# fedelopez77/sympa

Measured on AMD Instinct MI355X. Metric: pairwise Siegel distances/sec (upper, riem, n=4), higher is better.
Workload: dtype f64; 1 GPU; upper-riem-n4-b65536; manifold=upper, dist_metric=riem, dims=4, nodes=5041, table=trained, pairs=sampled, launch=fused, api=Model.forward_batches(Model.prepare_batches(list of K batches)), streams=1, parallelism=pairs sharded rank::1, table replicated, no collective, steps_per_launch=32

## Files before the change

__graft_entry__.py:

```python
import os
import subprocess
import sys

ROOT = os.path.dirname(os.path.abspath(__file__))
CSRC = os.path.join(ROOT, "sympa_amd", "csrc")
HOSTSIM = os.path.join(ROOT, "tests", "hostsim")
if ROOT not in sys.path:
    sys.path.insert(0, ROOT)


def _stale(target, sources):
    if not os.path.exists(target):
        return True
    t = os.path.getmtime(target)
    return any(os.path.getmtime(s) > t for s in sources)


INSTANCE_LIST = "siegel_bwd_instances.hpp"
INSTANCE_FAMILIES = {
    "COOP": ("siegel_bwd_coop_instance.hip", "siegel_bwd_coop_{model}_{n}_{form}"),
    "HALF": ("siegel_bwd_half_instance.hip", "siegel_bwd_half_{model}_{n}_{form}"),
    "SPLIT_SPECTRAL": ("siegel_bwd_split_instance.hip", "siegel_bwd_split_spectral_{model}_{n}"),
    "SPLIT_GRADIENT": ("siegel_bwd_split_instance.hip", "siegel_bwd_split_gradient_{model}_{n}_{form}"),
    "ONE_LANE": ("siegel_bwd_one_lane_instance.hip", "siegel_bwd_n{n}_{model}_{form}"),
}


def bwd_instances():
    import re
    out = []
    for line in open(os.path.join(CSRC, INSTANCE_LIST)):
        if line.startswith("SYMPA_BWD_"):
            m = re.fullmatch(r"SYMPA_BWD_([A-Z_]+)\(([a-z]+), (\d+)(?:, ([a-z]+))?\)\n", line)
            if not m or m.group(1) not in INSTANCE_FAMILIES or \
                    (m.group(4) is None) != ("{form}" not in INSTANCE_FAMILIES[m.group(1)][1]):
                raise ValueError(f"{INSTANCE_LIST}: cannot read the line {line!r}")
            out.append((m.group(1), m.group(2), int(m.group(3)), m.group(4)))
    return out


def hip_units():
    sources = {src for src, _ in INSTANCE_FAMILIES.values()}
    units = [(f, f, []) for f in os.listdir(CSRC) if f.endswith(".hip") and f not in sources]
    for family, model, n, form in bwd_instances():
        src, name = INSTANCE_FAMILIES[family]
        defines = [f"-DSYMPA_INST_MODEL={model}", f"-DSYMPA_INST_N={n}"] + ([f"-DSYMPA_INST_FORM={form}"] if form else [])
        units.append((name.format(model=model, n=n, form=form), src, defines))
    return sorted(units)


def build_hip(force=False):
    import shutil
    import tempfile
    from concurrent.futures import ThreadPoolExecutor
    sys.path.insert(0, os.path.join(ROOT, "tools"))
    import asm_stats
    import check_dpp_hazards
    import dma_reload_check
    import json
    so = os.path.join(CSRC, "libsympa_hip.so")
    units = hip_units()

    def obj_name(u):
        return (u[:-4] if u.endswith(".hip") else u) + ".o"
    headers = [os.path.join(CSRC, f) for f in os.listdir(CSRC) if f.endswith(".hpp")]
    headers.append(os.path.join(ROOT, "include", "sympa_hip.h"))
    flags = ["--offload-arch=gfx950", "-O3", "-std=c++17", "-fPIC"]
    unit_flags = {"siegel_dist_big.hip": ["-mllvm", "-enable-misched=0"],
                  "siegel_dist_big_dual.hip": ["-mllvm", "-enable-misched=0"],
                  "siegel_packed.hip": ["-mllvm", "-enable-misched=0"]}
    stats_units = ("siegel_dist.hip", "siegel_dist_big.hip", "siegel_packed.hip", "spd.hip")
    stats_path = os.path.join(CSRC, "asm_stats.json")
    try:
        stats = json.load(open(stats_path))
    except (OSError, ValueError):
        stats = {}
    report_path = os.path.join(CSRC, "dpp_hazard_report.txt")
    report = {}
    if os.path.exists(report_path):
        for line in open(report_path):
            parts = line.split()
            if len(parts) >= 2 and not line.startswith("#"):
                report[parts[0]] = line.strip()

    dma = {}

    def dma_note(u):
        return f"; {dma[u][0]} LDS-DMA instructions, {dma[u][1]} behind a scratch reload" if u in dma else ""

    def compile_checked(u, src, extra):
        tmp = tempfile.mkdtemp(prefix="sympa_build_")
        try:
            obj = os.path.join(tmp, obj_name(u))
            subprocess.check_call(["hipcc"] + flags + unit_flags.get(u, []) + extra + ["-c", "--save-temps=obj", "-o", obj, src], cwd=CSRC,
                                  stderr=subprocess.DEVNULL)
            asm = [os.path.join(tmp, f) for f in os.listdir(tmp) if f.endswith("gfx950.s")]
            assert len(asm) == 1, f"{u}: expected one gfx950 assembly file, got {asm}"
            total, bad = check_dpp_hazards.check_file(asm[0])
            dma[u] = dma_reload_check.totals(asm[0])
            if u in stats_units:
                stats[u] = asm_stats.kernel_flop_mix(asm[0])
            shutil.move(obj, os.path.join(CSRC, obj_name(u)))
            return total, bad
        finally:
            shutil.rmtree(tmp, ignore_errors=True)

    retries = [(["-DSYMPA_COOP_NOP_IN_ASM"], "SYMPA_COOP_NOP_IN_ASM")]

    def compile_unit(unit):
        u, src, defines = unit
        src, obj = os.path.join(CSRC, src), os.path.join(CSRC, obj_name(u))
        if force or u not in report or "LDS-DMA" not in report[u] or (u in stats_units and u not in stats) or \
                _stale(obj, [src] + headers):
            total, bad = compile_checked(u, src, defines)
            if bad:
                first = bad[0]
                print(f"[build] {u}: DPP hazard in the generated code ({first[1]}  ->  {first[2]})", flush=True)
                for extra, label in retries:
                    total, bad2 = compile_checked(u, src, defines + extra)
                    if not bad2:
                        report[u] = f"{u} {total} DPP instructions, {len(bad)} hazards -> rebuilt with {label}, clean" + dma_note(u)
                        break
                else:
                    raise RuntimeError(f"{u}: DPP hazard even with SYMPA_COOP_NOP_IN_ASM: {bad2[0]}")
            else:
                report[u] = f"{u} {total} DPP instructions, clean" + dma_note(u)
        return obj

    with ThreadPoolExecutor(max_workers=min(8, len(units))) as ex:
        objs = list(ex.map(compile_unit, units))
    with open(report_path, "w") as f:
        f.write("# tools/check_dpp_hazards.py and tools/dma_reload_check.py over the gfx950 assembly of every translation unit "
                "(written by build())\n")
        for u, _, _ in units:
            f.write(report[u] + "\n")
    with open(stats_path, "w") as f:
        json.dump({u: stats[u] for u in stats_units if u in stats}, f, indent=1, sort_keys=True)
    if force or _stale(so, objs):
        subprocess.check_call(["hipcc"] + flags + ["-shared", "-o", so] + objs, cwd=CSRC)
    return so


def build_torch_binding(force=False):
    import sysconfig
    import torch
    from torch.utils import cpp_extension as ce
    src = os.path.join(CSRC, "torch_binding.cpp")
    out = os.path.join(ROOT, "sympa_amd", "_fast" + sysconfig.get_config_var("EXT_SUFFIX"))
    stamp = out + ".torch_version"
    built_for = open(stamp).read().strip() if os.path.exists(stamp) else ""
    want = f"{torch.__version__} cxx11abi={int(torch.compiled_with_cxx11_abi())}"
    if not (force or built_for != want or _stale(out, [src, os.path.join(ROOT, "include", "sympa_hip.h")])):
        return out
    tl = os.path.join(os.path.dirname(torch.__file__), "lib")
    cmd = ["g++", "-O2", "-std=c++17", "-fPIC", "-shared", "-D__HIP_PLATFORM_AMD__=1", "-DUSE_ROCM=1",
           "-DTORCH_EXTENSION_NAME=_fast", "-DTORCH_API_INCLUDE_EXTENSION_H",
           f"-D_GLIBCXX_USE_CXX11_ABI={int(torch.compiled_with_cxx11_abi())}",
           "-I" + sysconfig.get_paths()["include"], "-I/opt/rocm/include"] + ["-I" + p for p in ce.include_paths()] + \
          [src, "-o", out, "-L" + tl, "-lc10", "-lc10_hip", "-ltorch", "-ltorch_cpu", "-ltorch_hip", "-ltorch_python",
           "-Wl,-rpath," + tl]
    subprocess.check_call(cmd, cwd=ROOT)
    with open(stamp, "w") as f:
        f.write(want + "\n")
    return out


def build_hostsim(force=False):
    so = os.path.join(HOSTSIM, "libsympa_hostsim.so")
    srcs = [os.path.join(HOSTSIM, "hostsim.cpp"), os.path.join(CSRC, "siegel_math.hpp"),
            os.path.join(CSRC, "siegel_math_bwd.hpp"), os.path.join(CSRC, "siegel_math_bwd_split.hpp"),
            os.path.join(CSRC, "siegel_table_math.hpp"),
            os.path.join(CSRC, "siegel_math_generic.hpp"), os.path.join(CSRC, "spd_math.hpp"),
            os.path.join(CSRC, "spd_math_bwd.hpp"), os.path.join(CSRC, "tridiag_invit.hpp")]
    if force or _stale(so, srcs):
        subprocess.check_call(["g++", "-O2", "-std=c++17", "-shared", "-fPIC", "-o", so, srcs[0]], cwd=HOSTSIM)
    return so


def build() -> None:
    build_hip()
    try:
        build_torch_binding()
    except (subprocess.CalledProcessError, OSError, ImportError) as e:
        print(f"[build] thin torch binding NOT built ({e!r}); the ctypes binding serves Model.forward", flush=True)
    build_hostsim()
    import sympa_amd
    from sympa_amd import _lib
    lib = _lib.load()
    assert lib.sympa_max_dims() >= 8
    print("built:", lib.sympa_version().decode())


def smoke() -> None:
    import torch
    build_hip()
    from oracle import siegel_oracle as so
    from sympa_amd import ops
    from sympa_amd.model import Model

    assert torch.cuda.is_available(), "smoke() needs a GPU"
    dev = torch.device("cuda:0")
    g = torch.Generator().manual_seed(7)
    n, N, b = 4, 97, 500
    for model in ("upper", "bounded"):
        class A:
            manifold, metric, dims, num_points = model, "riem", n, N
            scale_coef, scale_init, train_scale = 1.0, 1.0, False
        m = Model(A)
        with torch.no_grad():
            x = 0.3 * torch.randn(N, n, n, generator=g); x = 0.5 * (x + x.transpose(-1, -2))
            a = 0.3 * torch.randn(N, n, n, generator=g); y = torch.matrix_exp(0.5 * (a + a.transpose(-1, -2)))
            pts = torch.stack((x, 0.5 * (y + y.transpose(-1, -2))), 1)
            if model == "bounded":
                pts = so.to_symmetric(so.cayley_transform(pts))
            m.embeddings.embeds.data = pts
        m = m.to(dev)
        trip = torch.stack((torch.randint(0, N, (b,), generator=g), torch.randint(0, N, (b,), generator=g),
                            torch.randint(1, 9, (b,), generator=g)), 1)
        with torch.no_grad():
            got = m(trip.to(dev)).cpu()
        ops.check_status(dev)
        want = so.model_forward(pts, trip, model, "riem")
        rel = (((got - want).abs() - 1e-12).clamp_min(0) / want.abs().clamp_min(1e-300)).max().item()
        raw_abs = (got - want).abs().max().item()
        nz = want.abs() > 1e-9
        raw_rel = ((got - want).abs()[nz] / want.abs()[nz]).max().item()
        assert rel < 1e-8, f"{model}: HIP vs oracle rel err {rel}"
        print(f"smoke {model}: b={b} n={n} HIP vs oracle: max abs err {raw_abs:.2e}, max rel err {raw_rel:.2e} "
              f"(over the {int(nz.sum())} pairs with d > 1e-9), {rel:.2e} after the 1e-12 absolute floor")
    n8, N8 = 8, 61

    class A8:
        manifold, metric, dims, num_points = "upper", "riem", n8, N8
        scale_coef, scale_init, train_scale = 1.0, 1.0, False
    m = Model(A8)
    with torch.no_grad():
        x = 0.3 * torch.randn(N8, n8, n8, generator=g); x = 0.5 * (x + x.transpose(-1, -2))
        a = 0.2 * torch.randn(N8, n8, n8, generator=g); y = torch.matrix_exp(0.5 * (a + a.transpose(-1, -2)))
        pts = torch.stack((x, 0.5 * (y + y.transpose(-1, -2))), 1)
        m.embeddings.embeds.data = pts
    m = m.to(dev)
    trips = [torch.stack((torch.randint(0, N8, (bb,), generator=g), torch.randint(0, N8, (bb,), generator=g)), 1) for bb in (4100, 130, 1)]
    with torch.no_grad():
        outs = [o.cpu() for o in m.forward_batches([t.to(dev) for t in trips])]
    ops.check_status(dev)
    assert m.packed_table() is not None and m.packed_table().repacks == 1, "the packed path did not run"
    rel = 0.0
    for t, o in zip(trips, outs):
        want = so.model_forward(pts, t, "upper", "riem")
        rel = max(rel, (((o - want).abs() - 1e-12).clamp_min(0) / want.abs().clamp_min(1e-300)).max().item())
    assert rel < 1e-8, f"packed n = 8: HIP vs oracle rel err {rel}"
    print(f"smoke upper n={n8} packed list form (3 batches, {sum(t.shape[0] for t in trips)} pairs): HIP vs oracle max rel err {rel:.2e}")


if __name__ == "__main__":
    build()
    if len(sys.argv) > 1 and sys.argv[1] == "smoke":
        smoke()
```

sympa_amd/csrc/siegel_math.hpp:

```cpp
#pragma once

#include <cmath>
#include <cstdint>

#if defined(__HIPCC__)
#define SYMPA_HD __host__ __device__ __forceinline__
#else
#define SYMPA_HD inline
#endif

#ifndef SYMPA_UNROLL
#define SYMPA_UNROLL _Pragma("unroll")
#endif

namespace sympa {

enum Model : int { MODEL_UPPER = 0, MODEL_BOUNDED = 1, MODEL_DUAL = 2 };
enum Metric : int { METRIC_RIEM = 0, METRIC_FONE = 1, METRIC_FINF = 2, METRIC_FMIN = 3, METRIC_WSUM = 4 };

enum StatusBit : int { ST_NOT_PD = 1, ST_NONFINITE = 2, ST_BAD_INDEX = 4, ST_NO_CONVERGENCE = 8 };

#if defined(__HIP_DEVICE_COMPILE__)
SYMPA_HD bool wave_all(bool p) { return __all(p ? 1 : 0) != 0; }
SYMPA_HD double seed_rsq(double x) { return __builtin_amdgcn_rsq(x); }
SYMPA_HD double seed_rcp(double x) { return __builtin_amdgcn_rcp(x); }
SYMPA_HD double d_frexp_mant(double x) { return __builtin_amdgcn_frexp_mant(x); }
SYMPA_HD int d_frexp_exp(double x) { return __builtin_amdgcn_frexp_exp(x); }
#else
SYMPA_HD bool wave_all(bool p) { return p; }
SYMPA_HD double seed_rsq(double x) { return (1.0 / std::sqrt(x)) * (1.0 + 4.0e-8); }
SYMPA_HD double seed_rcp(double x) { return (1.0 / x) * (1.0 - 4.0e-8); }
SYMPA_HD double d_frexp_mant(double x) { int e; return std::frexp(x, &e); }
SYMPA_HD int d_frexp_exp(double x) { int e; (void)std::frexp(x, &e); return e; }
#endif
SYMPA_HD double d_fma(double a, double b, double c) { return __builtin_fma(a, b, c); }
SYMPA_HD bool d_finite(double x) { return fabs(x) <= 1.79e308; }

SYMPA_HD double d_rsqrt(double x) {
    const double y = seed_rsq(x);
    const double e = d_fma(-(x * y), y, 1.0);
    return d_fma(y, e * d_fma(0.375, e, 0.5), y);
}
SYMPA_HD double d_rcp(double x) {
    const double y = seed_rcp(x);
    const double e = d_fma(-x, y, 1.0);
    return d_fma(y, d_fma(e, e, e), y);
}
constexpr double TINY = 1e-300;
SYMPA_HD double d_sqrt(double x) { return x * d_rsqrt(x + TINY); }

SYMPA_HD double d_log1p(double u) {
    const double x = 1.0 + u;
    double m = d_frexp_mant(x);
    int k = d_frexp_exp(x);
    const bool lowhalf = m < 0.70710678118654752440;
    m = lowhalf ? 2.0 * m : m;
    k = lowhalf ? k - 1 : k;
    const bool small = u < 0.4;
    const double f = small ? u : m - 1.0;
    const double kd = small ? 0.0 : (double)k;
    const double s = f * d_rcp(2.0 + f);
    const double z = s * s;
    double r = 1.479819860511658591e-01;
    r = d_fma(r, z, 1.531383769920937332e-01);
    r = d_fma(r, z, 1.818357216161805012e-01);
    r = d_fma(r, z, 2.222219843214978396e-01);
    r = d_fma(r, z, 2.857142874366239149e-01);
    r = d_fma(r, z, 3.999999999940941908e-01);
    r = d_fma(r, z, 6.666666666666735130e-01);
    r = r * z;
    const double l = d_fma(-s, f - r, f);
    return d_fma(kd, 6.93147180559945286227e-01, l);
}

SYMPA_HD double d_atan2_pos(double s, double c) {
    const bool swap = s > c;
    const double num = swap ? c : s;
    const double den = swap ? s : c;
    const bool big = num > 0.41421356237309503 * den;
    const double xn = big ? num - den : num;
    const double xd = big ? num + den : den;
    const double x = xn * d_rcp(xd);
    const double z = x * x;
    const double w = z * z;
    double s1 = 1.62858201153657823623e-02;
    s1 = d_fma(s1, w, 4.97687799461593236017e-02);
    s1 = d_fma(s1, w, 6.66107313738753120669e-02);
    s1 = d_fma(s1, w, 9.09088713343650656196e-02);
    s1 = d_fma(s1, w, 1.42857142725034663711e-01);
    s1 = d_fma(s1, w, 3.33333333333329318027e-01);
    s1 = s1 * z;
    double s2 = -3.65315727442169155270e-02;
    s2 = d_fma(s2, w, -5.83357013379057348645e-02);
    s2 = d_fma(s2, w, -7.69187620504482999495e-02);
    s2 = d_fma(s2, w, -1.11111104054623557880e-01);
    s2 = d_fma(s2, w, -1.99999999998764832476e-01);
    s2 = s2 * w;
    double a = d_fma(-x, s1 + s2, x);
    a = big ? 7.85398163397448278999e-01 + (a + 3.06161699786838301793e-17) : a;
    return swap ? 1.57079632679489655800e+00 + (6.12323399573676603587e-17 - a) : a;
}

template <int N>
struct CMat {
    double re[N][N];
    double im[N][N];
};

template <int N, bool COMPLEX>
struct Tri {
    double re[N][N];
    double im[N][N];
    double rdiag[N];
};

template <int N>
SYMPA_HD void load_point(const double* __restrict__ p, CMat<N>& z) {
SYMPA_UNROLL
    for (int i = 0; i < N; ++i) {
SYMPA_UNROLL
        for (int j = 0; j < N; ++j) {
            z.re[i][j] = p[(i <= j) ? i * N + j : j * N + i];
            z.im[i][j] = p[N * N + ((i <= j) ? i * N + j : j * N + i)];
        }
    }
}

template <int N>
SYMPA_HD bool chol_real(const double (&y)[N][N], Tri<N, false>& l) {
    bool ok = true;
SYMPA_UNROLL
    for (int j = 0; j < N; ++j) {
        double s = y[j][j];
SYMPA_UNROLL
        for (int k = 0; k < j; ++k) s = d_fma(-l.re[j][k], l.re[j][k], s);
        ok = ok && (s > 0.0);
        const double r = d_rsqrt(s);
        l.rdiag[j] = r;
SYMPA_UNROLL
        for (int i = j + 1; i < N; ++i) {
            double t = y[j][i];
SYMPA_UNROLL
            for (int k = 0; k < j; ++k) t = d_fma(-l.re[i][k], l.re[j][k], t);
            l.re[i][j] = t * r;
        }
    }
    return ok;
}

template <bool PLUS>
SYMPA_HD double wwh_sign(double x) {
    if constexpr (PLUS) return x;
    else return -x;
}
template <int N, bool PLUS>
SYMPA_HD bool chol_id_pm_wwh(const CMat<N>& w, Tri<N, true>& c) {
    bool ok = true;
SYMPA_UNROLL
    for (int j = 0; j < N; ++j) {
        double s = 1.0;
SYMPA_UNROLL
        for (int l = 0; l < N; ++l) {
            s = d_fma(wwh_sign<PLUS>(w.re[j][l]), w.re[j][l], s);
            s = d_fma(wwh_sign<PLUS>(w.im[j][l]), w.im[j][l], s);
        }
SYMPA_UNROLL
        for (int k = 0; k < j; ++k) {
            s = d_fma(-c.re[j][k], c.re[j][k], s);
            s = d_fma(-c.im[j][k], c.im[j][k], s);
        }
        ok = ok && (s > 0.0);
        const double r = d_rsqrt(s);
        c.rdiag[j] = r;
SYMPA_UNROLL
        for (int i = j + 1; i < N; ++i) {
            double tr = 0.0, ti = 0.0;
SYMPA_UNROLL
            for (int l = 0; l < N; ++l) {
                tr = d_fma(wwh_sign<PLUS>(w.re[i][l]), w.re[j][l], tr);
                tr = d_fma(wwh_sign<PLUS>(w.im[i][l]), w.im[j][l], tr);
                ti = d_fma(wwh_sign<PLUS>(w.im[i][l]), w.re[j][l], ti);
                ti = d_fma(-wwh_sign<PLUS>(w.re[i][l]), w.im[j][l], ti);
            }
SYMPA_UNROLL
            for (int k = 0; k < j; ++k) {
                tr = d_fma(-c.re[i][k], c.re[j][k], tr);
                tr = d_fma(-c.im[i][k], c.im[j][k], tr);
                ti = d_fma(-c.im[i][k], c.re[j][k], ti);
                ti = d_fma(c.re[i][k], c.im[j][k], ti);
            }
            c.re[i][j] = tr * r;
            c.im[i][j] = ti * r;
        }
    }
    return ok;
}

template <int N>
SYMPA_HD bool chol_id_minus_wwh(const CMat<N>& w, Tri<N, true>& c) { return chol_id_pm_wwh<N, false>(w, c); }
template <int N>
SYMPA_HD bool chol_id_plus_wwh(const CMat<N>& w, Tri<N, true>& c) { return chol_id_pm_wwh<N, true>(w, c); }
template <int N, int MODEL>
SYMPA_HD bool chol_model_factor(const CMat<N>& w, Tri<N, true>& c) {
    static_assert(MODEL == MODEL_BOUNDED || MODEL == MODEL_DUAL, "the upper model factors Im z (chol_real)");
    return chol_id_pm_wwh<N, MODEL == MODEL_DUAL>(w, c);
}

template <int N, bool COMPLEX>
SYMPA_HD void solve_left(const Tri<N, COMPLEX>& l, CMat<N>& e) {
SYMPA_UNROLL
    for (int c = 0; c < N; ++c) {
SYMPA_UNROLL
        for (int i = 0; i < N; ++i) {
            double tr = e.re[i][c], ti = e.im[i][c];
SYMPA_UNROLL
            for (int k = 0; k < i; ++k) {
                tr = d_fma(-l.re[i][k], e.re[k][c], tr);
                ti = d_fma(-l.re[i][k], e.im[k][c], ti);
                if (COMPLEX) {
                    tr = d_fma(l.im[i][k], e.im[k][c], tr);
                    ti = d_fma(-l.im[i][k], e.re[k][c], ti);
                }
            }
            e.re[i][c] = tr * l.rdiag[i];
            e.im[i][c] = ti * l.rdiag[i];
        }
    }
}

template <int N, bool COMPLEX>
SYMPA_HD void solve_right_t(const Tri<N, COMPLEX>& l, CMat<N>& e) {
SYMPA_UNROLL
    for (int r = 0; r < N; ++r) {
SYMPA_UNROLL
        for (int j = 0; j < N; ++j) {
            double tr = e.re[r][j], ti = e.im[r][j];
SYMPA_UNROLL
            for (int k = 0; k < j; ++k) {
                tr = d_fma(-e.re[r][k], l.re[j][k], tr);
                ti = d_fma(-e.im[r][k], l.re[j][k], ti);
                if (COMPLEX) {
                    tr = d_fma(e.im[r][k], l.im[j][k], tr);
                    ti = d_fma(-e.re[r][k], l.im[j][k], ti);
                }
            }
            e.re[r][j] = tr * l.rdiag[j];
            e.im[r][j] = ti * l.rdiag[j];
        }
    }
}

template <int N>
struct Herm {
    double d[N];
    double re[N][N];
    double im[N][N];
};

template <int N>
SYMPA_HD void gram(const CMat<N>& e, Herm<N>& h) {
SYMPA_UNROLL
    for (int j = 0; j < N; ++j) {
        double s = 0.0;
SYMPA_UNROLL
        for (int i = 0; i < N; ++i) {
            s = d_fma(e.re[i][j], e.re[i][j], s);
            s = d_fma(e.im[i][j], e.im[i][j], s);
        }
        h.d[j] = s;
SYMPA_UNROLL
        for (int k = j + 1; k < N; ++k) {
            double tr = 0.0, ti = 0.0;
SYMPA_UNROLL
            for (int i = 0; i < N; ++i) {
                tr = d_fma(e.re[i][j], e.re[i][k], tr);
                tr = d_fma(e.im[i][j], e.im[i][k], tr);
                ti = d_fma(e.re[i][j], e.im[i][k], ti);
                ti = d_fma(-e.im[i][j], e.re[i][k], ti);
            }
            h.re[j][k] = tr;
            h.im[j][k] = ti;
        }
    }
}

template <int N>
SYMPA_HD void jacobi_rotate(Herm<N>& h, const int p, const int q) {
        {
        const double br = h.re[p][q], bi = h.im[p][q];
        const double a2 = d_fma(br, br, bi * bi);
        const double delta = h.d[q] - h.d[p];
        const double ad = fabs(delta) + 1e-150;
        const double qr = d_rsqrt(d_fma(ad, ad, 4.0 * a2));
        const double c2 = d_fma(0.5 * ad, qr, 0.5);
        const double ic = d_rsqrt(c2);
        const double c = c2 * ic;
        const double cu = copysign(qr, delta) * ic;
        const double ua2 = (cu * ic) * a2;
        const double wr = cu * br, wi = cu * bi;
        h.d[p] -= ua2;
        h.d[q] += ua2;
        h.re[p][q] = 0.0;
        h.im[p][q] = 0.0;
SYMPA_UNROLL
        for (int k = 0; k < N; ++k) {
            if (k == p || k == q) continue;
            double xr, xi, yr, yi;
            if (k < p) { xr = h.re[k][p]; xi = h.im[k][p]; } else { xr = h.re[p][k]; xi = -h.im[p][k]; }
            if (k < q) { yr = h.re[k][q]; yi = h.im[k][q]; } else { yr = h.re[q][k]; yi = -h.im[q][k]; }
            const double nxr = d_fma(-wi, yi, d_fma(-wr, yr, c * xr));
            const double nxi = d_fma(wi, yr, d_fma(-wr, yi, c * xi));
            const double nyr = d_fma(-wi, xi, d_fma(wr, xr, c * yr));
            const double nyi = d_fma(wi, xr, d_fma(wr, xi, c * yi));
            if (k < p) { h.re[k][p] = nxr; h.im[k][p] = nxi; } else { h.re[p][k] = nxr; h.im[p][k] = -nxi; }
            if (k < q) { h.re[k][q] = nyr; h.im[k][q] = nyi; } else { h.re[q][k] = nyr; h.im[q][k] = -nyi; }
        }
        }
}

template <int N>
SYMPA_HD void jacobi_sweep(Herm<N>& h) {
    if (N == 4) {
        jacobi_rotate<N>(h, 0, 1); jacobi_rotate<N>(h, 2, 3);
        jacobi_rotate<N>(h, 0, 2); jacobi_rotate<N>(h, 1, 3);
        jacobi_rotate<N>(h, 0, 3); jacobi_rotate<N>(h, 1, 2);
    } else {
SYMPA_UNROLL
        for (int p = 0; p < N - 1; ++p) {
SYMPA_UNROLL
            for (int q = p + 1; q < N; ++q) jacobi_rotate<N>(h, p, q);
        }
    }
}

template <int N>
SYMPA_HD void herm_norms(const Herm<N>& h, double& off2, double& diag2) {
    off2 = 0.0;
    diag2 = 0.0;
SYMPA_UNROLL
    for (int j = 0; j < N; ++j) {
        diag2 = d_fma(h.d[j], h.d[j], diag2);
SYMPA_UNROLL
        for (int k = j + 1; k < N; ++k) {
            off2 = d_fma(h.re[j][k], h.re[j][k], off2);
            off2 = d_fma(h.im[j][k], h.im[j][k], off2);
        }
    }
}

template <int N>
SYMPA_HD void jacobi_diag_update(Herm<N>& h, const int p, const int q) {
    const double br = h.re[p][q], bi = h.im[p][q];
    const double a2 = d_fma(br, br, bi * bi);
    const double delta = h.d[q] - h.d[p];
    const double ad = fabs(delta) + 1e-150;
    const double qr = d_rsqrt(d_fma(ad, ad, 4.0 * a2));
    const double c2 = d_fma(0.5 * ad, qr, 0.5);
    const double ua2 = (copysign(qr, delta) * a2) * (2.0 - c2);
    h.d[p] -= ua2;
    h.d[q] += ua2;
}

template <int N>
SYMPA_HD void jacobi_final_sweep(Herm<N>& h) {
SYMPA_UNROLL
    for (int p = 0; p < N - 1; ++p) {
SYMPA_UNROLL
        for (int q = p + 1; q < N; ++q) jacobi_diag_update<N>(h, p, q);
    }
}

template <int N> constexpr double finish_t2() { return N <= 4 ? 1e-3 : 1e-8; }
template <int N> constexpr double finish_off2() { return N <= 4 ? 1e-4 : 1e-12; }
constexpr double FINISH_NEGLIGIBLE2 = 1e-24;

template <int N>
SYMPA_HD bool jacobi_can_finish(const Herm<N>& h) {
    double diag2 = 0.0;
SYMPA_UNROLL
    for (int j = 0; j < N; ++j) diag2 = d_fma(h.d[j], h.d[j], diag2);
    const double floor2 = FINISH_NEGLIGIBLE2 * diag2;
    double off2 = 0.0;
    bool ok = true;
SYMPA_UNROLL
    for (int p = 0; p < N - 1; ++p) {
SYMPA_UNROLL
        for (int q = p + 1; q < N; ++q) {
            const double a2 = d_fma(h.re[p][q], h.re[p][q], h.im[p][q] * h.im[p][q]);
            const double delta = h.d[q] - h.d[p];
            off2 += a2;
            ok = ok && !(a2 > fmax(finish_t2<N>() * delta * delta, floor2));
        }
    }
    return ok && !(off2 > finish_off2<N>() * diag2);
}

constexpr int JACOBI_MAX_SWEEPS = 16;
template <int N>
constexpr int jacobi_blind_sweeps() { return N <= 2 ? 1 : (N <= 4 ? 3 : 4); }

template <int N>
SYMPA_HD bool herm_eigenvalues_jacobi(Herm<N>& h) {
    if (N == 1) return true;
SYMPA_UNROLL
    for (int sweep = 0; sweep < jacobi_blind_sweeps<N>(); ++sweep) jacobi_sweep<N>(h);
    if (N == 2) return true;
    bool conv = false;
    for (int sweep = jacobi_blind_sweeps<N>(); sweep < JACOBI_MAX_SWEEPS; ++sweep) {
        conv = jacobi_can_finish<N>(h);
        if (wave_all(conv)) break;
        jacobi_sweep<N>(h);
    }
    jacobi_final_sweep<N>(h);
    return conv;
}

template <int N>
SYMPA_HD void herm_get(const Herm<N>& h, int i, int j, double& re, double& im) {
    if (i < j) { re = h.re[i][j]; im = h.im[i][j]; } else { re = h.re[j][i]; im = -h.im[j][i]; }
}

template <int N>
SYMPA_HD void herm_tridiagonalize(Herm<N>& h, double (&a)[N], double (&b2)[N]) {
SYMPA_UNROLL
    for (int k = 0; k < N - 2; ++k) {
        constexpr int dummy = 0; (void)dummy;
        double vr[N], vi[N];
        double sig2 = 0.0;
SYMPA_UNROLL
        for (int i = k + 1; i < N; ++i) {
            herm_get<N>(h, i, k, vr[i], vi[i]);
            if (i > k + 1) sig2 = d_fma(vr[i], vr[i], d_fma(vi[i], vi[i], sig2));
        }
        const double x02 = d_fma(vr[k + 1], vr[k + 1], vi[k + 1] * vi[k + 1]);
        const double n2 = x02 + sig2;
        a[k] = h.d[k];
        b2[k] = n2;
        const double nx = d_sqrt(n2);
        const double ix0 = d_rsqrt(x02 + TINY);
        const double ax0 = x02 * ix0;
        const bool x0zero = !(x02 > 0.0);
        const double pr = x0zero ? 1.0 : vr[k + 1] * ix0, pi = x0zero ? 0.0 : vi[k + 1] * ix0;
        vr[k + 1] = pr * (ax0 + nx);
        vi[k + 1] = pi * (ax0 + nx);
        const double beta = (sig2 > 0.0) ? d_rcp(nx * (nx + ax0)) : 0.0;
        double qr[N], qi[N];
        double kk = 0.0;
SYMPA_UNROLL
        for (int i = k + 1; i < N; ++i) {
            double tr = h.d[i] * vr[i], ti = h.d[i] * vi[i];
SYMPA_UNROLL
            for (int j = k + 1; j < N; ++j) {
                if (j == i) continue;
                double ar, ai;
                herm_get<N>(h, i, j, ar, ai);
                tr = d_fma(ar, vr[j], tr); tr = d_fma(-ai, vi[j], tr);
                ti = d_fma(ar, vi[j], ti); ti = d_fma(ai, vr[j], ti);
            }
            qr[i] = beta * tr; qi[i] = beta * ti;
            kk = d_fma(vr[i], qr[i], kk); kk = d_fma(vi[i], qi[i], kk);
        }
        kk *= 0.5 * beta;
SYMPA_UNROLL
        for (int i = k + 1; i < N; ++i) { qr[i] = d_fma(-kk, vr[i], qr[i]); qi[i] = d_fma(-kk, vi[i], qi[i]); }
SYMPA_UNROLL
        for (int i = k + 1; i < N; ++i) {
            h.d[i] -= 2.0 * d_fma(vr[i], qr[i], vi[i] * qi[i]);
SYMPA_UNROLL
            for (int j = i + 1; j < N; ++j) {
                double tr = d_fma(vr[i], qr[j], vi[i] * qi[j]);
                double ti = d_fma(vi[i], qr[j], -vr[i] * qi[j]);
                tr = d_fma(qr[i], vr[j], d_fma(qi[i], vi[j], tr));
                ti = d_fma(qi[i], vr[j], d_fma(-qr[i], vi[j], ti));
                h.re[i][j] -= tr;
                h.im[i][j] -= ti;
            }
        }
    }
    a[N - 2] = h.d[N - 2];
    a[N - 1] = h.d[N - 1];
    b2[N - 2] = d_fma(h.re[N - 2][N - 1], h.re[N - 2][N - 1], h.im[N - 2][N - 1] * h.im[N - 2][N - 1]);
    b2[N - 1] = 0.0;
}

template <int N>
SYMPA_HD bool tridiag_ql(double (&d)[N], double (&e2)[N]) {
    constexpr double TOL = 1.3e-32;
    int l = 0;
    bool done = false;
    for (int iter = 0; iter < 40 * N; ++iter) {
SYMPA_UNROLL
        for (int i = 0; i < N - 1; ++i)
            if (e2[i] <= TOL * fabs(d[i] * d[i + 1]) + 1e-290) e2[i] = 0.0;
SYMPA_UNROLL
        for (int i = 0; i < N - 1; ++i)
            if (l == i && e2[i] == 0.0) l = i + 1;
        done = l >= N - 1;
        if (wave_all(done)) break;
        int m = N - 1;
SYMPA_UNROLL
        for (int i = N - 2; i >= 0; --i)
            if (i >= l && e2[i] == 0.0) m = i;
        double dl = 0.0, dl1 = 0.0, el = 1.0, dm = 0.0;
SYMPA_UNROLL
        for (int i = 0; i < N; ++i) {
            if (i == l) dl = d[i];
            if (i == l + 1) dl1 = d[i];
            if (i == m) dm = d[i];
            if (i < N - 1 && i == l) el = e2[i];
        }
        if (done) el = 1.0;
        const double irte = d_rsqrt(el);
        const double rte = el * irte;
        double sg = 0.5 * (dl1 - dl) * irte;
        const double rr = d_sqrt(d_fma(sg, sg, 1.0));
        const double sigma = dl - rte * d_rcp(sg + copysign(rr, sg));
        double c = 1.0, sn = 0.0, gamma = dm - sigma, p = gamma * gamma;
SYMPA_UNROLL
        for (int i = N - 2; i >= 0; --i) {
            if (!done && i >= l && i <= m - 1) {
                const double bb = e2[i];
                const double r = p + bb;
                if (i < N - 2 && i != m - 1) e2[i + 1] = sn * r;
                const double oldc = c;
                const double ir = d_rcp(r);
                c = p * ir;
                sn = bb * ir;
                const double oldgam = gamma;
                const double alpha = d[i];
                gamma = d_fma(c, alpha - sigma, -sn * oldgam);
                d[i + 1] = oldgam + (alpha - gamma);
                p = (c != 0.0) ? gamma * gamma * d_rcp(c) : oldc * bb;
            }
        }
        if (!done) {
SYMPA_UNROLL
            for (int i = 0; i < N; ++i) {
                if (i == l) d[i] = sigma + gamma;
                if (i < N - 1 && i == l) e2[i] = sn * p;
            }
        }
    }
    return done;
}

constexpr double QL_DEFLATE_TOL = 1e-20;
constexpr double QL_DEFLATE_TOL_EXACT = 1.3e-32;
SYMPA_HD bool ql_negligible(double e2, double da, double db) { return !(e2 > 1.3e-32 * fabs(da * db) + 1e-290); }
template <bool VALUES_ONLY>
SYMPA_HD bool ql_deflated(double e2, double da, double db, double tol = QL_DEFLATE_TOL) {
    return !(e2 > (VALUES_ONLY ? tol : 1.3e-32) * fabs(da * db) + 1e-290);
}
SYMPA_HD double ql_deflate_tol_for(int metric, bool wants_vvd) {
    return (metric == METRIC_RIEM || metric == METRIC_FONE) && !wants_vvd ? QL_DEFLATE_TOL : QL_DEFLATE_TOL_EXACT;
}

template <int N, int L, bool VALUES_ONLY>
SYMPA_HD bool tridiag_ql_stage(double (&d)[N], double (&e2)[N], const double tol) {
    bool conv = false;
    for (int it = 0; it < 60; ++it) {
        conv = ql_deflated<VALUES_ONLY>(e2[L], d[L], d[L + 1], tol);
        if (wave_all(conv)) break;
        double dl = d[L], dl1 = d[L + 1], el = e2[L];
        bool idle = conv;
        e2[L] = conv ? 0.0 : e2[L];
        if constexpr (L + 1 <= N - 2) {
            const bool c1 = ql_deflated<VALUES_ONLY>(e2[L + 1], d[L + 1], d[L + 2], tol);
            dl = idle ? d[L + 1] : dl;
            dl1 = idle ? d[L + 2] : dl1;
            el = idle ? e2[L + 1] : el;
            idle = idle && c1;
            e2[L + 1] = idle ? 0.0 : e2[L + 1];
            if constexpr (L + 2 <= N - 2) {
                const bool c2 = ql_deflated<VALUES_ONLY>(e2[L + 2], d[L + 2], d[L + 3], tol);
                dl = idle ? d[L + 2] : dl;
                dl1 = idle ? d[L + 3] : dl1;
                el = idle ? e2[L + 2] : el;
                idle = idle && c2;
                e2[L + 2] = idle ? 0.0 : e2[L + 2];
            }
        }
        el = idle ? 1.0 : el;
        const double irte = d_rsqrt(el);
        const double rte = el * irte;
        const double sg = 0.5 * (dl1 - dl) * irte;
        const double rr = d_sqrt(d_fma(sg, sg, 1.0));
        double sigma = dl - rte * d_rcp(sg + copysign(rr, sg));
        sigma = idle ? dl : sigma;
        double c = 1.0, sn = 0.0, gamma = d[N - 1] - sigma, p = gamma * gamma;
SYMPA_UNROLL
        for (int i = N - 2; i >= L; --i) {
            const double bb = e2[i];
            const double r = p + bb;
            if (i != N - 2) e2[i + 1] = sn * r;
            const double oldc = c;
            const double rs = fmax(r, TINY);
            const double ir = d_rcp(rs);
            c = (p + (rs - r)) * ir;
            sn = bb * ir;
            const double oldgam = gamma;
            const double alpha = d[i];
            gamma = d_fma(c, alpha - sigma, -sn * oldgam);
            d[i + 1] = oldgam + (alpha - gamma);
            const double pn = gamma * gamma * d_rcp(c);
            const double pz = oldc * bb;
            p = (c != 0.0) ? pn : pz;
        }
        e2[L] = sn * p;
        d[L] = sigma + gamma;
    }
    return conv;
}

template <int N, int L = 0, bool VALUES_ONLY = false>
SYMPA_HD bool tridiag_ql_lockstep(double (&d)[N], double (&e2)[N], const double tol = QL_DEFLATE_TOL) {
    if constexpr (L >= N - 1) {
        return true;
    } else {
        const bool here = tridiag_ql_stage<N, L, VALUES_ONLY>(d, e2, tol);
        const bool rest = tridiag_ql_lockstep<N, L + 1, VALUES_ONLY>(d, e2, tol);
        return here && rest;
    }
}

template <int N>
SYMPA_HD bool herm_eigenvalues(Herm<N>& h, const double ql_tol = QL_DEFLATE_TOL) {
    if constexpr (N <= 4) {
        return herm_eigenvalues_jacobi<N>(h);
    } else {
        double a[N], b2[N];
        herm_tridiagonalize<N>(h, a, b2);
        const bool ok = tridiag_ql_lockstep<N, 0, true>(a, b2, ql_tol);
SYMPA_UNROLL
        for (int i = 0; i < N; ++i) h.d[i] = a[i];
        return ok;
    }
}

SYMPA_HD double vvd_from_sinh2(double lambda, double inv_eps) {
    double u = 2.0 * (lambda + d_sqrt(d_fma(lambda, lambda, lambda)));
    if (u >= inv_eps - 1.0) {
        const double d = d_sqrt(lambda * d_rcp(1.0 + lambda));
        const double clamped = d_fma(1.0 + d, inv_eps, -1.0);
        u = u < clamped ? u : clamped;
    }
    return d_log1p(u);
}

SYMPA_HD double vvd_from_sin2(double lambda) {
    const double lam = fmin(lambda, 1.0);
    return d_atan2_pos(d_sqrt(lam), d_sqrt(1.0 - lam));
}

template <int N>
SYMPA_HD void sort_ascending(double (&v)[N]) {
SYMPA_UNROLL
    for (int round = 0; round < N; ++round) {
SYMPA_UNROLL
        for (int i = (round & 1); i + 1 < N; i += 2) {
            const double lo = fmin(v[i], v[i + 1]);
            const double hi = fmax(v[i], v[i + 1]);
            v[i] = lo;
            v[i + 1] = hi;
        }
    }
}

template <int N>
SYMPA_HD double reduce_metric(double (&v)[N], int metric, const double* __restrict__ w) {
    double acc = 0.0;
    if (metric == METRIC_RIEM) {
SYMPA_UNROLL
        for (int i = 0; i < N; ++i) acc = d_fma(v[i], v[i], acc);
        return d_sqrt(acc);
    }
    if (metric == METRIC_FONE) {
SYMPA_UNROLL
        for (int i = 0; i < N; ++i) acc += v[i];
        return acc;
    }
    if (metric == METRIC_FINF) {
        acc = v[0];
SYMPA_UNROLL
        for (int i = 1; i < N; ++i) acc = fmax(acc, v[i]);
        return acc;
    }
    sort_ascending<N>(v);
    if (metric == METRIC_FMIN) {
SYMPA_UNROLL
        for (int i = 0; i < N; ++i) acc = d_fma(2.0 * i, v[i], acc);
        return acc;
    }
SYMPA_UNROLL
    for (int i = 0; i < N; ++i) acc = d_fma(fmax(w[i], 0.0), v[i], acc);
    return acc;
}

template <int N, int MODEL>
SYMPA_HD double distance_from_h(Herm<N>& h, const bool ok, int metric, const double* __restrict__ w,
                                double inv_eps, double* __restrict__ vvd, int& status) {
    const bool conv = herm_eigenvalues<N>(h, ql_deflate_tol_for(metric, vvd != nullptr));

    const double scale = (MODEL == MODEL_UPPER) ? 0.25 : 1.0;
    double v[N];
    bool finite = true;
SYMPA_UNROLL
    for (int i = 0; i < N; ++i) {
        finite = finite && d_finite(h.d[i]);
        if constexpr (MODEL == MODEL_DUAL) v[i] = vvd_from_sin2(fmax(h.d[i], 0.0));
        else v[i] = vvd_from_sinh2(fmax(h.d[i], 0.0) * scale, inv_eps);
    }
    if (!finite) {
SYMPA_UNROLL
        for (int i = 0; i < N; ++i) v[i] = __builtin_nan("");
    }

    if (vvd != nullptr) {
        sort_ascending<N>(v);
SYMPA_UNROLL
        for (int i = 0; i < N; ++i) vvd[i] = v[i];
    }
    double out = reduce_metric<N>(v, metric, w);
    if (!finite) out = __builtin_nan("");
    if (!ok) status |= ST_NOT_PD;
    if (!conv) status |= ST_NO_CONVERGENCE;
    if (!d_finite(out)) status |= ST_NONFINITE;
    return out;
}

template <int N, int MODEL>
SYMPA_HD double distance_from_e(const CMat<N>& e, const bool ok, int metric, const double* __restrict__ w,
                                double inv_eps, double* __restrict__ vvd, int& status) {
    Herm<N> h;
    gram<N>(e, h);
    return distance_from_h<N, MODEL>(h, ok, metric, w, inv_eps, vvd, status);
}

template <int N, int MODEL>
SYMPA_HD double pair_distance_mats(const CMat<N>& z1, const CMat<N>& z2, int metric, const double* __restrict__ w,
                                   double inv_eps, double* __restrict__ vvd, int& status) {
    CMat<N> e;
    bool ok;
    {
        if constexpr (MODEL == MODEL_UPPER) {
            Tri<N, false> l1, l2;
            ok = chol_real<N>(z1.im, l1);
            ok = chol_real<N>(z2.im, l2) && ok;
SYMPA_UNROLL
            for (int i = 0; i < N; ++i)
SYMPA_UNROLL
                for (int j = 0; j < N; ++j) {
                    e.re[i][j] = z2.re[i][j] - z1.re[i][j];
                    e.im[i][j] = z2.im[i][j] - z1.im[i][j];
                }
            solve_left<N, false>(l1, e);
            solve_right_t<N, false>(l2, e);
        } else {
            Tri<N, true> c1, c2;
            ok = chol_model_factor<N, MODEL>(z1, c1);
            ok = chol_model_factor<N, MODEL>(z2, c2) && ok;
SYMPA_UNROLL
            for (int i = 0; i < N; ++i)
SYMPA_UNROLL
                for (int j = 0; j < N; ++j) {
                    e.re[i][j] = z2.re[i][j] - z1.re[i][j];
                    e.im[i][j] = z2.im[i][j] - z1.im[i][j];
                }
            solve_left<N, true>(c1, e);
            solve_right_t<N, true>(c2, e);
        }
    }
    return distance_from_e<N, MODEL>(e, ok, metric, w, inv_eps, vvd, status);
}

template <int N, int MODEL>
struct PointPack {
    static constexpr int TRI = N * (N + 1) / 2;
    static constexpr int LOW = N * (N - 1) / 2;
    static constexpr int OFF_IM = TRI;
    static constexpr int OFF_DIAG = 2 * TRI;
    static constexpr int OFF_LRE = 2 * TRI + N;
    static constexpr int OFF_LIM = 2 * TRI + N + LOW;
    static constexpr int LEN = 2 * TRI + N + (MODEL == MODEL_UPPER ? LOW : 2 * LOW);
};
SYMPA_HD constexpr int tri_index(int n, int i, int j) { return i * n - i * (i - 1) / 2 + (j - i); }
SYMPA_HD constexpr int low_index(int i, int j) { return i * (i - 1) / 2 + j; }

template <int N, int MODEL>
SYMPA_HD bool pack_point(const CMat<N>& z, double (&p)[PointPack<N, MODEL>::LEN]) {
    using P = PointPack<N, MODEL>;
SYMPA_UNROLL
    for (int i = 0; i < N; ++i)
SYMPA_UNROLL
        for (int j = i; j < N; ++j) {
            p[tri_index(N, i, j)] = z.re[i][j];
            p[P::OFF_IM + tri_index(N, i, j)] = z.im[i][j];
        }
    Tri<N, MODEL != MODEL_UPPER> l;
    bool ok;
    if constexpr (MODEL == MODEL_UPPER) ok = chol_real<N>(z.im, l);
    else ok = chol_model_factor<N, MODEL>(z, l);
    double ar[N][N], ai[N][N];
SYMPA_UNROLL
    for (int j = 0; j < N; ++j) {
        ar[j][j] = l.rdiag[j];
        ai[j][j] = 0.0;
SYMPA_UNROLL
        for (int i = j + 1; i < N; ++i) {
            double tr = 0.0, ti = 0.0;
SYMPA_UNROLL
            for (int k = j; k < i; ++k) {
                tr = d_fma(l.re[i][k], ar[k][j], tr);
                if (MODEL != MODEL_UPPER) {
                    tr = d_fma(-l.im[i][k], ai[k][j], tr);
                    ti = d_fma(l.re[i][k], ai[k][j], ti);
                    ti = d_fma(l.im[i][k], ar[k][j], ti);
                }
            }
            ar[i][j] = -tr * l.rdiag[i];
            ai[i][j] = -ti * l.rdiag[i];
        }
    }
SYMPA_UNROLL
    for (int i = 0; i < N; ++i) {
        p[P::OFF_DIAG + i] = ar[i][i];
SYMPA_UNROLL
        for (int j = 0; j < i; ++j) {
            p[P::OFF_LRE + low_index(i, j)] = ar[i][j];
            if constexpr (MODEL != MODEL_UPPER) p[P::OFF_LIM + low_index(i, j)] = ai[i][j];
        }
    }
    return ok;
}

template <int N, int MODEL, bool DIFF = false, class P1, class P2>
SYMPA_HD void e_from_packed(const P1& p1, const P2& p2, CMat<N>& e) {
    using P = PointPack<N, MODEL>;
    constexpr bool CPLX = MODEL != MODEL_UPPER;
SYMPA_UNROLL
    for (int i = 0; i < N; ++i)
SYMPA_UNROLL
        for (int j = i; j < N; ++j) {
            const double xr = DIFF ? p2[tri_index(N, i, j)] : p2[tri_index(N, i, j)] - p1[tri_index(N, i, j)];
            const double xi = DIFF ? p2[P::OFF_IM + tri_index(N, i, j)]
                                   : p2[P::OFF_IM + tri_index(N, i, j)] - p1[P::OFF_IM + tri_index(N, i, j)];
            e.re[i][j] = xr; e.im[i][j] = xi;
            e.re[j][i] = xr; e.im[j][i] = xi;
        }
SYMPA_UNROLL
    for (int rr = 0; rr < N; ++rr) {
        const int r = N - 1 - rr;
        const double dg = p1[P::OFF_DIAG + r];
        double lr[N], li[N];
SYMPA_UNROLL
        for (int k = 0; k < r; ++k) {
            lr[k] = p1[P::OFF_LRE + low_index(r, k)];
            if constexpr (CPLX) li[k] = p1[P::OFF_LIM + low_index(r, k)];
        }
SYMPA_UNROLL
        for (int c = 0; c < N; ++c) {
            double xr = dg * e.re[r][c], xi = dg * e.im[r][c];
SYMPA_UNROLL
            for (int k = 0; k < r; ++k) {
                xr = d_fma(lr[k], e.re[k][c], xr);
                xi = d_fma(lr[k], e.im[k][c], xi);
                if constexpr (CPLX) {
                    xr = d_fma(-li[k], e.im[k][c], xr);
                    xi = d_fma(li[k], e.re[k][c], xi);
                }
            }
            e.re[r][c] = xr;
            e.im[r][c] = xi;
        }
    }
SYMPA_UNROLL
    for (int cc = 0; cc < N; ++cc) {
        const int c = N - 1 - cc;
        const double dg = p2[P::OFF_DIAG + c];
        double lr[N], li[N];
SYMPA_UNROLL
        for (int k = 0; k < c; ++k) {
            lr[k] = p2[P::OFF_LRE + low_index(c, k)];
            if constexpr (CPLX) li[k] = p2[P::OFF_LIM + low_index(c, k)];
        }
SYMPA_UNROLL
        for (int r = 0; r < N; ++r) {
            double xr = e.re[r][c] * dg, xi = e.im[r][c] * dg;
SYMPA_UNROLL
            for (int k = 0; k < c; ++k) {
                xr = d_fma(e.re[r][k], lr[k], xr);
                xi = d_fma(e.im[r][k], lr[k], xi);
                if constexpr (CPLX) {
                    xr = d_fma(-e.im[r][k], li[k], xr);
                    xi = d_fma(e.re[r][k], li[k], xi);
                }
            }
            e.re[r][c] = xr;
            e.im[r][c] = xi;
        }
    }
}

template <int N, int MODEL>
SYMPA_HD double pair_distance(const double* __restrict__ p1, const double* __restrict__ p2, int metric,
                              const double* __restrict__ w, double inv_eps, double* __restrict__ vvd, int& status) {
    CMat<N> z1, z2;
    load_point<N>(p1, z1);
    load_point<N>(p2, z2);
    return pair_distance_mats<N, MODEL>(z1, z2, metric, w, inv_eps, vvd, status);
}

}
```

Measured before the change: 14.99 billion pairs/s.

## Fuse paired Jacobi rotations into rounds and exploit known-zero entries

Replaces the six separate 4x4 complex Jacobi rotations per sweep with three rounds, each applying two disjoint rotations together to the 2x2 cross block with a shared cosine product. Within a round it skips arithmetic on entries already known to be zero from the previous round or sweep. The final diagonal-only sweep now reuses pivot magnitudes computed in the convergence check and uses a cheaper rational formula, skipping pivots that are known zero. This cuts FLOPs and rsqrt calls in the eigenvalue loop, at the cost of relying on exact zero-pattern assumptions, which changes rounding slightly. A host-side test library build is also added.

```diff
diff --git a/__graft_entry__.py b/__graft_entry__.py
--- a/__graft_entry__.py
+++ b/__graft_entry__.py
@@ -174,6 +174,10 @@
             os.path.join(CSRC, "spd_math_bwd.hpp"), os.path.join(CSRC, "tridiag_invit.hpp")]
     if force or _stale(so, srcs):
         subprocess.check_call(["g++", "-O2", "-std=c++17", "-shared", "-fPIC", "-o", so, srcs[0]], cwd=HOSTSIM)
+    eig = os.path.join(HOSTSIM, "libsympa_jacobi_eig.so")
+    eig_srcs = [os.path.join(HOSTSIM, "jacobi_eig.cpp"), os.path.join(CSRC, "siegel_math.hpp")]
+    if force or _stale(eig, eig_srcs):
+        subprocess.check_call(["g++", "-O2", "-std=c++17", "-shared", "-fPIC", "-o", eig, eig_srcs[0]], cwd=HOSTSIM)
     return so
 
 
diff --git a/sympa_amd/csrc/siegel_math.hpp b/sympa_amd/csrc/siegel_math.hpp
--- a/sympa_amd/csrc/siegel_math.hpp
+++ b/sympa_amd/csrc/siegel_math.hpp
@@ -285,6 +285,23 @@
 }
 
 template <int N>
+SYMPA_HD void jacobi_angle(const Herm<N>& h, const int p, const int q, double& c, double& tr, double& ti, double& ua2) {
+    const double br = h.re[p][q], bi = h.im[p][q];
+    const double a2 = d_fma(br, br, bi * bi);
+    const double delta = h.d[q] - h.d[p];
+    const double ad = fabs(delta) + 1e-150;
+    const double qr = d_rsqrt(d_fma(ad, ad, 4.0 * a2));
+    const double c2 = d_fma(0.5 * ad, qr, 0.5);
+    const double ic = d_rsqrt(c2);
+    c = c2 * ic;
+    const double cu = copysign(qr, delta) * ic;
+    const double uc = cu * ic;
+    ua2 = uc * a2;
+    tr = uc * br;
+    ti = uc * bi;
+}
+
+template <int N>
 SYMPA_HD void jacobi_rotate(Herm<N>& h, const int p, const int q) {
         {
         const double br = h.re[p][q], bi = h.im[p][q];
@@ -319,11 +336,75 @@
 }
 
 template <int N>
-SYMPA_HD void jacobi_sweep(Herm<N>& h) {
-    if (N == 4) {
-        jacobi_rotate<N>(h, 0, 1); jacobi_rotate<N>(h, 2, 3);
-        jacobi_rotate<N>(h, 0, 2); jacobi_rotate<N>(h, 1, 3);
-        jacobi_rotate<N>(h, 0, 3); jacobi_rotate<N>(h, 1, 2);
+SYMPA_HD void herm_get(const Herm<N>& h, int i, int j, double& re, double& im) {
+    if (i < j) { re = h.re[i][j]; im = h.im[i][j]; } else { re = h.re[j][i]; im = -h.im[j][i]; }
+}
+template <int N>
+SYMPA_HD void herm_set(Herm<N>& h, int i, int j, double re, double im) {
+    if (i < j) { h.re[i][j] = re; h.im[i][j] = im; } else { h.re[j][i] = re; h.im[j][i] = -im; }
+}
+
+enum RoundZeros : int { ROUND_FULL = 0, ROUND_DIAG = 1, ROUND_ANTI = 2 };
+
+template <int ZEROS>
+SYMPA_HD void jacobi_round(Herm<4>& h, const int p, const int q, const int r, const int s) {
+    double ca, ar, ai, ua, cb, br, bi, ub;
+    jacobi_angle<4>(h, p, q, ca, ar, ai, ua);
+    jacobi_angle<4>(h, r, s, cb, br, bi, ub);
+    h.d[p] -= ua;
+    h.d[q] += ua;
+    h.d[r] -= ub;
+    h.d[s] += ub;
+    h.re[p][q] = 0.0;
+    h.im[p][q] = 0.0;
+    h.re[r][s] = 0.0;
+    h.im[r][s] = 0.0;
+    const double cc = ca * cb;
+    const int row[2] = {p, q}, col[2] = {r, s};
+    double mr[2][2], mi[2][2];
+SYMPA_UNROLL
+    for (int i = 0; i < 2; ++i) {
+SYMPA_UNROLL
+        for (int j = 0; j < 2; ++j) herm_get<4>(h, row[i], col[j], mr[i][j], mi[i][j]);
+    }
+    double pr[2][2], pi[2][2];
+SYMPA_UNROLL
+    for (int j = 0; j < 2; ++j) {
+        if ((ZEROS == ROUND_DIAG && j == 0) || (ZEROS == ROUND_ANTI && j == 1)) {
+            pr[0][j] = d_fma(ai, mi[1][j], -ar * mr[1][j]);
+            pi[0][j] = d_fma(-ai, mr[1][j], -ar * mi[1][j]);
+            pr[1][j] = mr[1][j];
+            pi[1][j] = mi[1][j];
+        } else if ((ZEROS == ROUND_DIAG && j == 1) || (ZEROS == ROUND_ANTI && j == 0)) {
+            pr[0][j] = mr[0][j];
+            pi[0][j] = mi[0][j];
+            pr[1][j] = d_fma(ai, mi[0][j], ar * mr[0][j]);
+            pi[1][j] = d_fma(-ai, mr[0][j], ar * mi[0][j]);
+        } else {
+            pr[0][j] = d_fma(ai, mi[1][j], d_fma(-ar, mr[1][j], mr[0][j]));
+            pi[0][j] = d_fma(-ai, mr[1][j], d_fma(-ar, mi[1][j], mi[0][j]));
+            pr[1][j] = d_fma(ai, mi[0][j], d_fma(ar, mr[0][j], mr[1][j]));
+            pi[1][j] = d_fma(-ai, mr[0][j], d_fma(ar, mi[0][j], mi[1][j]));
+        }
+    }
+SYMPA_UNROLL
+    for (int i = 0; i < 2; ++i) {
+        const double q0r = d_fma(-bi, pi[i][1], d_fma(-br, pr[i][1], pr[i][0]));
+        const double q0i = d_fma(bi, pr[i][1], d_fma(-br, pi[i][1], pi[i][0]));
+        const double q1r = d_fma(-bi, pi[i][0], d_fma(br, pr[i][0], pr[i][1]));
+        const double q1i = d_fma(bi, pr[i][0], d_fma(br, pi[i][0], pi[i][1]));
+        herm_set<4>(h, row[i], col[0], cc * q0r, cc * q0i);
+        herm_set<4>(h, row[i], col[1], cc * q1r, cc * q1i);
+    }
+}
+
+template <int N>
+SYMPA_HD void jacobi_sweep(Herm<N>& h, const bool after_sweep = false) {
+    if constexpr (N == 4) {
+        if (after_sweep) jacobi_round<ROUND_ANTI>(h, 0, 1, 2, 3);
+        else jacobi_round<ROUND_FULL>(h, 0, 1, 2, 3);
+        jacobi_round<ROUND_DIAG>(h, 0, 2, 1, 3);
+        jacobi_round<ROUND_ANTI>(h, 0, 3, 1, 2);
     } else {
 SYMPA_UNROLL
         for (int p = 0; p < N - 1; ++p) {
@@ -349,25 +430,44 @@
 }
 
 template <int N>
-SYMPA_HD void jacobi_diag_update(Herm<N>& h, const int p, const int q) {
-    const double br = h.re[p][q], bi = h.im[p][q];
-    const double a2 = d_fma(br, br, bi * bi);
+SYMPA_HD void jacobi_diag_update(Herm<N>& h, const int p, const int q, const double a2) {
     const double delta = h.d[q] - h.d[p];
     const double ad = fabs(delta) + 1e-150;
-    const double qr = d_rsqrt(d_fma(ad, ad, 4.0 * a2));
-    const double c2 = d_fma(0.5 * ad, qr, 0.5);
-    const double ua2 = (copysign(qr, delta) * a2) * (2.0 - c2);
+    const double ua2 = (a2 * delta) * d_rcp(d_fma(ad, ad, a2));
     h.d[p] -= ua2;
     h.d[q] += ua2;
 }
 
+template <int N> constexpr int herm_pivots() { return N > 1 ? N * (N - 1) / 2 : 1; }
+
+template <int N>
+SYMPA_HD void herm_pivot_a2(const Herm<N>& h, double (&a2)[herm_pivots<N>()]) {
+    int k = 0;
+SYMPA_UNROLL
+    for (int p = 0; p < N - 1; ++p) {
+SYMPA_UNROLL
+        for (int q = p + 1; q < N; ++q, ++k) a2[k] = d_fma(h.re[p][q], h.re[p][q], h.im[p][q] * h.im[p][q]);
+    }
+}
+
+template <int N, bool AFTER_SWEEP>
+SYMPA_HD void jacobi_final_sweep(Herm<N>& h, const double (&a2)[herm_pivots<N>()]) {
+    int k = 0;
+SYMPA_UNROLL
+    for (int p = 0; p < N - 1; ++p) {
+SYMPA_UNROLL
+        for (int q = p + 1; q < N; ++q, ++k) {
+            if (AFTER_SWEEP && N == 4 && p + q == 3) continue;
+            jacobi_diag_update<N>(h, p, q, a2[k]);
+        }
+    }
+}
+
 template <int N>
 SYMPA_HD void jacobi_final_sweep(Herm<N>& h) {
-SYMPA_UNROLL
-    for (int p = 0; p < N - 1; ++p) {
-SYMPA_UNROLL
-        for (int q = p + 1; q < N; ++q) jacobi_diag_update<N>(h, p, q);
-    }
+    double a2[herm_pivots<N>()];
+    herm_pivot_a2<N>(h, a2);
+    jacobi_final_sweep<N, false>(h, a2);
 }
 
 template <int N> constexpr double finish_t2() { return N <= 4 ? 1e-3 : 1e-8; }
@@ -375,21 +475,22 @@
 constexpr double FINISH_NEGLIGIBLE2 = 1e-24;
 
 template <int N>
-SYMPA_HD bool jacobi_can_finish(const Herm<N>& h) {
+SYMPA_HD bool jacobi_can_finish(const Herm<N>& h, double (&a2)[herm_pivots<N>()]) {
     double diag2 = 0.0;
 SYMPA_UNROLL
     for (int j = 0; j < N; ++j) diag2 = d_fma(h.d[j], h.d[j], diag2);
     const double floor2 = FINISH_NEGLIGIBLE2 * diag2;
+    herm_pivot_a2<N>(h, a2);
     double off2 = 0.0;
     bool ok = true;
+    int k = 0;
 SYMPA_UNROLL
     for (int p = 0; p < N - 1; ++p) {
 SYMPA_UNROLL
-        for (int q = p + 1; q < N; ++q) {
-            const double a2 = d_fma(h.re[p][q], h.re[p][q], h.im[p][q] * h.im[p][q]);
+        for (int q = p + 1; q < N; ++q, ++k) {
             const double delta = h.d[q] - h.d[p];
-            off2 += a2;
-            ok = ok && !(a2 > fmax(finish_t2<N>() * delta * delta, floor2));
+            off2 += a2[k];
+            ok = ok && !(a2[k] > fmax(finish_t2<N>() * delta * delta, floor2));
         }
     }
     return ok && !(off2 > finish_off2<N>() * diag2);
@@ -403,22 +504,21 @@
 SYMPA_HD bool herm_eigenvalues_jacobi(Herm<N>& h) {
     if (N == 1) return true;
 SYMPA_UNROLL
-    for (int sweep = 0; sweep < jacobi_blind_sweeps<N>(); ++sweep) jacobi_sweep<N>(h);
+    for (int sweep = 0; sweep < jacobi_blind_sweeps<N>(); ++sweep) jacobi_sweep<N>(h, sweep > 0);
     if (N == 2) return true;
     bool conv = false;
-    for (int sweep = jacobi_blind_sweeps<N>(); sweep < JACOBI_MAX_SWEEPS; ++sweep) {
-        conv = jacobi_can_finish<N>(h);
+    double a2[herm_pivots<N>()];
+    int sweep = jacobi_blind_sweeps<N>();
+    for (; sweep < JACOBI_MAX_SWEEPS; ++sweep) {
+        conv = jacobi_can_finish<N>(h, a2);
         if (wave_all(conv)) break;
-        jacobi_sweep<N>(h);
-    }
-    jacobi_final_sweep<N>(h);
+        jacobi_sweep<N>(h, true);
+    }
+    if (sweep == JACOBI_MAX_SWEEPS) herm_pivot_a2<N>(h, a2);
+    jacobi_final_sweep<N, true>(h, a2);
     return conv;
 }
 
-template <int N>
-SYMPA_HD void herm_get(const Herm<N>& h, int i, int j, double& re, double& im) {
-    if (i < j) { re = h.re[i][j]; im = h.im[i][j]; } else { re = h.re[j][i]; im = -h.im[j][i]; }
-}
 
 template <int N>
 SYMPA_HD void herm_tridiagonalize(Herm<N>& h, double (&a)[N], double (&b2)[N]) {
```

Result: faster. 16.09 billion pairs/s, median of 6 (+7.3%).
